# jeff-regier/Celeste.jl

Measured on AMD Instinct MI355X. Metric: sources/sec (ELBO value+gradient+Hessian+KL per target source), higher is better.
Workload: dtype f64; 1 GPU; BASELINE.json configs[2]: synthetic 2048x1489x5 SDSS-size field, 2000 star+galaxy sources, fp64, Sa=1 with value-only neighbours, psf_K=2; gather_backend=none, neighbor_links_rank0=3526

## Files before the change

### celeste.jl_amd/csrc/celeste_abi.hip

```cpp
#include <hip/hip_runtime.h>
#include <algorithm>
#include <atomic>
#include <cmath>
#include <cstdio>
#include <cstdlib>
#include <cstring>
#include <mutex>
#include <unordered_map>
#include <vector>

#include "elbo_kernels.h"
#include "optim_kernels.h"
#include "fused_kernels.h"
#include "host_tables.h"

struct celeste_group;

#define EVAL_FUSED_MAX 32

#define HIP_TRY(expr)                                                                    \
    do {                                                                                 \
        hipError_t e__ = (expr);                                                         \
        if (e__ != hipSuccess) {                                                         \
            fprintf(stderr, "celeste_mi355x: %s failed: %s (%s:%d)\n", #expr,            \
                    hipGetErrorString(e__), __FILE__, __LINE__);                         \
            return CELESTE_ERR_HIP;                                                      \
        }                                                                                \
    } while (0)

static hipError_t celeste_device_malloc(void **p, size_t bytes) {
    hipError_t e = (hipMalloc)(p, bytes);
    static const bool poison = [] { const char *v = getenv("CELESTE_POISON"); return v && atoi(v) != 0; }();
    if (e == hipSuccess && poison) {
        e = hipMemset(*p, 0xFF, bytes);
        if (e == hipSuccess) e = hipDeviceSynchronize();
    }
    return e;
}
#define hipMalloc(p, bytes) celeste_device_malloc((void **)(p), (bytes))

struct StreamPool {
    std::mutex mu;
    std::vector<hipStream_t> idle[16];
};
static StreamPool &stream_pool() { static StreamPool *p = new StreamPool(); return *p; }
static hipError_t stream_acquire(int device, hipStream_t *out) {
    *out = nullptr;
    if (device >= 0 && device < 16) {
        StreamPool &sp = stream_pool();
        std::lock_guard<std::mutex> lk(sp.mu);
        if (!sp.idle[device].empty()) { *out = sp.idle[device].back(); sp.idle[device].pop_back(); return hipSuccess; }
    }
    return hipStreamCreateWithFlags(out, hipStreamNonBlocking);
}
static void stream_retire(int device, hipStream_t s) {
    if (!s) return;
    if (hipStreamSynchronize(s) == hipSuccess && device >= 0 && device < 16) {
        static const size_t cap = [] { const char *e = getenv("CELESTE_STREAM_POOL_MAX"); return e ? (size_t)std::max(0, atoi(e)) : (size_t)32; }();
        StreamPool &sp = stream_pool();
        std::lock_guard<std::mutex> lk(sp.mu);
        if (sp.idle[device].size() < cap) { sp.idle[device].push_back(s); return; }
    } else (void)hipGetLastError();
    (void)hipStreamDestroy(s);
}

struct PinnedPool {
    std::mutex mu;
// ... 37 lines not shown


struct celeste_images {
    int device = 0;
    int N = 0;
    std::vector<DevImage> h_images;
    std::vector<void *> plane_allocs;
    DevImage *d_images = nullptr;
    std::atomic<int> refs{1};
};

static void images_release(celeste_images *im) {
    if (!im || im->refs.fetch_sub(1) != 1) return;
    (void)hipSetDevice(im->device);
    for (void *p : im->plane_allocs) (void)hipFree(p);
    if (im->d_images) (void)hipFree(im->d_images);
    delete im;
}

struct celeste_ctx {
    int device = 0;
    celeste_images *imgs = nullptr;
    hipStream_t stream = nullptr;
    hipStream_t copy_stream = nullptr;
    bool copy_stream_checked = false;
    int N = 0, S = 0, K = 0, NC = 0, n_stamps = 0;
    int chunk_px = 256, CH = 1;
    int max_npx = 0;
    std::vector<DevPatch> h_patches;
    std::vector<int64_t> h_nbr_off;
    std::vector<int32_t> h_nbr_idx;
    DevImage *d_images = nullptr;
    DevPatch *d_patches = nullptr;
    double *d_coefs = nullptr;
    float *d_coefs_f = nullptr;
    uint8_t *d_bitmaps = nullptr;
    int64_t *d_nbr_off = nullptr;
    int32_t *d_nbr_idx = nullptr;
    PriorDev *d_prior = nullptr;
    SrcImg *d_srcimg = nullptr;
    Comp *d_comps = nullptr;
    SrcGeo *d_geo = nullptr;
    int64_t *d_val_off = nullptr;
    double2 *d_val = nullptr;
    int32_t *d_needed = nullptr;
    int32_t stamp = 0;
    std::vector<int32_t> h_vis_off, h_vis_img, h_vis_src;
    int32_t *d_vis_off = nullptr, *d_vis_img = nullptr, *d_vis_src = nullptr;
    int4 *d_value_items = nullptr;
    int4 *d_vitems_src = nullptr;
    int32_t *d_vitem_off = nullptr;
    std::vector<int32_t> h_vitem_off;
    std::vector<int32_t> h_vitem_tgt;
    int64_t n_value_items = 0;
    std::vector<struct celeste_targets *> lists;
    int32_t *d_prep_mark = nullptr;
    double *d_lg_sum = nullptr;
    int64_t *d_nv_base = nullptr;
    int32_t *d_nbr_vis = nullptr;
    int2 *d_items = nullptr;
    size_t items_cap = 0;
    std::vector<int32_t> h_src_chunks;
    std::vector<int64_t> h_top_chunks;
    int max_src_chunks = 0;
    int32_t *d_work = nullptr, *d_work_blk = nullptr, *d_work_total = nullptr;
    size_t work_cap = 0, work_blk_cap = 0;
    int M = 1;
    bool dense = false;
    int64_t V = 0;
    std::vector<int64_t> h_tile_off;
    int64_t *d_tile_off = nullptr;
    int64_t n_tiles = 0;
    int sum_tiles = 4, RCH = 1;
    double *d_rec = nullptr;
    double *d_acc_split = nullptr;
    size_t acc_split_cap = 0;
    double *d_acc = nullptr;
    size_t acc_cap = 0;
    int32_t *d_rec_off = nullptr;
    size_t rec_off_cap = 0;
    double *d_vp = nullptr;
    int32_t *d_targets = nullptr;
    double *d_v = nullptr, *d_d = nullptr, *d_h = nullptr;
    int64_t *d_cnt = nullptr;
    int32_t *d_status = nullptr;
    size_t stage_cap = 0;
    double *p_vp = nullptr;
    int32_t *p_targets = nullptr, *p_status = nullptr;
    double *p_v = nullptr, *p_d = nullptr, *p_h = nullptr;
    int64_t *p_cnt = nullptr;
    size_t pin_cap = 0;
    double *d_small_in = nullptr, *p_small_in = nullptr, *d_small_out = nullptr, *p_small_out = nullptr;
    static const int MAX_PARTS = 8;
    hipEvent_t part_done[MAX_PARTS] = {}, part_copied[MAX_PARTS] = {};
    struct OptBuffers {
        size_t cap = 0;
        double *d_vp = nullptr, *d_v = nullptr, *d_d = nullptr, *d_h = nullptr, *d_H = nullptr, *d_T = nullptr, *d_S = nullptr, *d_pos = nullptr;
        int32_t *d_targets = nullptr, *d_act[2] = {nullptr, nullptr}, *d_evt[2] = {nullptr, nullptr}, *d_count = nullptr,
                *d_st = nullptr;
        void *d_state = nullptr;
        static const int RING = 4;
        double *h_vp = nullptr;
        void *h_state = nullptr;
        int32_t *h_count = nullptr;
        hipEvent_t ev[RING] = {};
    } opt;
// ... 340 lines not shown
        std::vector<int64_t> base((size_t)c->S + 1, 0);
        for (int s = 0; s < c->S; ++s)
            base[s + 1] = base[s] + (int64_t)(c->h_vis_off[s + 1] - c->h_vis_off[s]) * (c->h_nbr_off[s + 1] - c->h_nbr_off[s]);
        std::vector<int32_t> nv((size_t)base[c->S]);
        for (int s = 0; s < c->S; ++s) {
            const int64_t K = c->h_nbr_off[s + 1] - c->h_nbr_off[s];
            for (int v = c->h_vis_off[s]; v < c->h_vis_off[s + 1]; ++v)
                for (int64_t q = 0; q < K; ++q)
                    nv[base[s] + (int64_t)(v - c->h_vis_off[s]) * K + q] = (int32_t)hv(c->h_nbr_idx[c->h_nbr_off[s] + q], c->h_vis_img[v]);
        }
        CTX_TRY(dev_upload(&c->d_nv_base, base.data(), base.size()));
        CTX_TRY(dev_upload(&c->d_nbr_vis, nv.data(), nv.size()));
    }
    {
        std::vector<int32_t> sorted(c->h_src_chunks);
        std::sort(sorted.begin(), sorted.end(), [](int32_t a, int32_t b) { return a > b; });
        c->h_top_chunks.assign((size_t)c->S + 1, 0);
        for (int s = 0; s < c->S; ++s) c->h_top_chunks[s + 1] = c->h_top_chunks[s] + sorted[s];
    }
    CTX_TRY(dev_upload<int32_t>(&c->d_work_total, nullptr, 1));
    {
        if (c->N > 0xffff) { celeste_ctx_destroy(c); return CELESTE_ERR_INVALID_ARG; }
        const int n_cls = c->chunk_px / 64;
        std::vector<std::vector<std::pair<int32_t, int32_t>>> by_len(n_cls);
        for (int s = 0; s < c->S; ++s)
            for (int64_t q = c->h_nbr_off[s]; q < c->h_nbr_off[s + 1]; ++q) {
                const int s2 = c->h_nbr_idx[q];
                for (int va = c->h_vis_off[s]; va < c->h_vis_off[s + 1]; ++va) {
                    const int n = c->h_vis_img[va];
                    const int64_t vb = hv(s2, n);
                    if (vb < 0) continue;
                    const DevPatch &a = c->h_patches[va], &b = c->h_patches[vb];
                    const int rh = std::min(a.off_h + a.H2, b.off_h + b.H2) - std::max(a.off_h, b.off_h);
                    const int rw = std::min(a.off_w + a.W2, b.off_w + b.W2 - 1) - std::max(a.off_w, b.off_w);
                    if (rh <= 0 || rw <= 0) continue;
                    const int npx = rh * rw, nch = (npx + c->chunk_px - 1) / c->chunk_px;
                    for (int ch = 0; ch < nch; ++ch) {
                        const int px = std::min(c->chunk_px, npx - ch * c->chunk_px);
                        by_len[n_cls - (px + 63) / 64].push_back({(int32_t)q, (int32_t)(n | (ch << 16))});
                    }
                }
            }
        std::vector<int32_t> link_src(c->h_nbr_idx.size());
        for (int s = 0; s < c->S; ++s)
            for (int64_t q = c->h_nbr_off[s]; q < c->h_nbr_off[s + 1]; ++q) link_src[q] = s;
        std::vector<int4> desc;
        for (auto &v : by_len)
            for (auto &e : v) {
                const int t = link_src[e.first], s2 = c->h_nbr_idx[e.first], n = e.second & 0xffff, ch = e.second >> 16;
                desc.push_back(make_int4((int)hv(s2, n), (int)hv(t, n), ch, t));
            }
        c->n_value_items = (int64_t)desc.size();
        c->h_vitem_tgt.resize(desc.size());
        for (size_t i = 0; i < desc.size(); ++i) c->h_vitem_tgt[i] = desc[i].w;
        CTX_TRY(dev_upload(&c->d_value_items, desc.data(), desc.size()));
        c->h_vitem_off.assign((size_t)c->S + 1, 0);
        for (auto &d : desc) c->h_vitem_off[(size_t)d.w + 1]++;
        for (int s = 0; s < c->S; ++s) c->h_vitem_off[s + 1] += c->h_vitem_off[s];
        {
            std::vector<int4> by_src(desc.size());
            std::vector<int32_t> fill(c->h_vitem_off.begin(), c->h_vitem_off.end() - 1);
            for (auto &d : desc) by_src[(size_t)fill[d.w]++] = d;
            CTX_TRY(dev_upload(&c->d_vitems_src, by_src.data(), by_src.size()));
            CTX_TRY(dev_upload(&c->d_vitem_off, c->h_vitem_off.data(), c->h_vitem_off.size()));
        }
        CTX_TRY(dev_upload<int32_t>(&c->d_prep_mark, nullptr, (size_t)c->S));
        if (hipMemset(c->d_prep_mark, 0, (size_t)c->S * sizeof(int32_t)) != hipSuccess) { celeste_ctx_destroy(c); return CELESTE_ERR_HIP; }
    }
    {
        c->h_tile_off.resize(c->h_patches.size());
        int64_t tot = 0;
        for (size_t q = 0; q < c->h_patches.size(); ++q) {
            c->h_tile_off[q] = tot;
            tot += ((int64_t)c->h_patches[q].H2 * c->h_patches[q].W2 + 63) / 64;
        }
        c->n_tiles = tot;
        if (const char *e = getenv("CELESTE_SUM_TILES")) if (atoi(e) > 0) c->sum_tiles = atoi(e);
        c->RCH = std::max(1, ((c->max_npx + 63) / 64 + c->sum_tiles - 1) / c->sum_tiles);
    }
    if (hipStreamSynchronize(nullptr) != hipSuccess) { celeste_ctx_destroy(c); return CELESTE_ERR_HIP; }
#undef CTX_TRY
    *out = c;
    return CELESTE_OK;
} ABI_CATCH

static void targets_free(struct celeste_targets *t);
extern "C" void celeste_ctx_destroy(celeste_ctx_t *c) {
    if (!c) return;
    (void)hipSetDevice(c->device);
    if (c->stream) (void)hipStreamSynchronize(c->stream);
    if (c->copy_stream) (void)hipStreamSynchronize(c->copy_stream);
    for (struct celeste_targets *t : c->lists) targets_free(t);
    c->lists.clear();
    void *ptrs[] = {c->d_patches, c->d_coefs, c->d_coefs_f, c->d_bitmaps, c->d_nbr_off, c->d_nbr_idx, c->d_prior,
                    c->d_srcimg, c->d_comps, c->d_geo, c->d_val_off, c->d_val, c->d_needed, c->d_vis_off, c->d_vis_img, c->d_vis_src, c->d_value_items, c->d_vitems_src, c->d_vitem_off, c->d_prep_mark, c->d_rec_off, c->d_lg_sum, c->d_nv_base, c->d_nbr_vis, c->d_items, c->d_work, c->d_work_blk, c->d_work_total, c->d_tile_off, c->d_rec, c->d_acc_split, c->d_acc, c->d_vp, c->d_targets, c->d_v, c->d_d, c->d_h,
                    c->d_cnt, c->d_status};
    for (void *p : ptrs) if (p) (void)hipFree(p);
    {
        auto &o = c->opt;
        void *optr[] = {o.d_vp, o.d_v, o.d_d, o.d_h, o.d_H, o.d_T, o.d_S, o.d_pos, o.d_targets, o.d_act[0], o.d_act[1], o.d_evt[0], o.d_evt[1],
                        o.d_count, o.d_st, o.d_state};
        for (void *q : optr) if (q) (void)hipFree(q);
        void *hptr[] = {o.h_vp, o.h_state, o.h_count};
        for (void *q : hptr) if (q) staging_free(q);
        for (int k = 0; k < celeste_ctx::OptBuffers::RING; ++k) if (o.ev[k]) (void)hipEventDestroy(o.ev[k]);
        auto &f = c->fused;
        void *fptr[] = {f.d_chunk_desc, f.d_tgt_rec, f.d_q_items, f.d_q_ctl, f.d_arrivals, f.d_saved};
// ... 264 lines not shown
    d_active_rank, c->d_items, c->M, c->d_work, c->d_work_total, c->d_nv_base, c->d_nbr_vis, c->d_rec_off, c->d_coefs_f
#define LAUNCH_PIXEL_T(MODE, R) hipLaunchKernelGGL((pixel_kernel<MODE, R>), grid, dim3(64), 0, stream, PIXEL_ARGS)
#define LAUNCH_PIXEL_M(MODE) hipLaunchKernelGGL((pixel_kernel<MODE, double, true>), grid, dim3(64), 0, stream, PIXEL_ARGS)
#define LAUNCH_PIXEL(MODE) do { if (flags & CELESTE_FLAG_FP32) LAUNCH_PIXEL_T(MODE, float); else LAUNCH_PIXEL_T(MODE, double); } while (0)
    if (d_active_rank) {
        if (flags & CELESTE_FLAG_HESS) LAUNCH_PIXEL_M(2);
        else if (derivs) LAUNCH_PIXEL_M(1);
        else LAUNCH_PIXEL_M(0);
    }
    else if (split) LAUNCH_PIXEL(3);
    else if (flags & CELESTE_FLAG_HESS) LAUNCH_PIXEL(2);
    else if (derivs) LAUNCH_PIXEL(1);
    else LAUNCH_PIXEL_T(0, double);
#undef LAUNCH_PIXEL
#undef LAUNCH_PIXEL_M
#undef PIXEL_ARGS
#undef LAUNCH_PIXEL_T
    if (c->timing) HIP_TRY(hipEventRecord(c->ev[2], stream));
    c->ev_split = 0;
    const int lift_nt = n_targets <= 1024 ? 512 : 256;
    bool lift7 = n_targets > 4096;
    if (const char *e = getenv("CELESTE_LIFT_WAVES")) lift7 = atoi(e) == 7;
#define LAUNCH_LIFT(...) do { if (lift7) hipLaunchKernelGGL(lift_kernel<7>, __VA_ARGS__); else hipLaunchKernelGGL(lift_kernel<8>, __VA_ARGS__); } while (0)
    if (split) {
        hipLaunchKernelGGL(record_sum_kernel, dim3((unsigned)((size_t)n_targets * c->M * c->RCH)), dim3(RSUM_NT), 0,
                           stream, c->d_patches, d_targets, c->d_tile_off, reinterpret_cast<const double2 *>(c->d_rec),
                           c->d_items, c->N, c->M, c->RCH, c->sum_tiles, c->d_acc_split, nullptr, c->d_work_total);
        if (c->timing) { HIP_TRY(hipEventRecord(c->ev[4], stream)); c->ev_split = 1; }
        LAUNCH_LIFT(dim3(n_targets), dim3(lift_nt), 0, stream, d_vp, c->d_images, c->d_patches, c->d_geo,
                           c->d_nbr_off, c->d_nbr_idx, d_targets, c->d_acc_split, c->d_prior, c->d_vis_off, c->d_vis_img, c->N, c->M,
                           c->RCH, c->sum_tiles * 64, flags,
                           d_v, d_d, d_h, d_counters, d_status, d_live, d_active_rank ? nullptr : c->d_lg_sum, nullptr, d_h_pos);
    } else
    LAUNCH_LIFT(dim3(n_targets), dim3(lift_nt), 0, stream, d_vp, c->d_images, c->d_patches, c->d_geo,
                       c->d_nbr_off, c->d_nbr_idx, d_targets, c->d_acc, c->d_prior, c->d_vis_off, c->d_vis_img, c->N, c->M, CH,
                       chunk_px, flags,
                       d_v, d_d, d_h, d_counters, d_status, d_live, d_active_rank ? nullptr : c->d_lg_sum, c->d_rec_off, d_h_pos);
#undef LAUNCH_LIFT
    if (c->timing) { HIP_TRY(hipEventRecord(c->ev[3], stream)); c->ev_valid = 1; }
    HIP_TRY(hipGetLastError());
    return CELESTE_OK;
}

struct celeste_targets {
    celeste_ctx_t *ctx = nullptr;
    int32_t n = 0;
    int G = 1;
    int32_t *d_targets = nullptr;
    int32_t *d_work = nullptr, *d_work_total = nullptr, *d_rec_off = nullptr;
    int2 *d_items = nullptr;
    int32_t *d_needed = nullptr;
    int32_t *d_visits = nullptr;
    int32_t *d_vitems = nullptr;
    int64_t n_visits = 0, n_vitems = 0;
    int64_t n_records = 0;
    int32_t n_work = 0;
};
static const int32_t LIST_STAMP = 1;

static void targets_free(celeste_targets *t) {
    if (!t) return;
    void *ptrs[] = {t->d_targets, t->d_work, t->d_work_total, t->d_rec_off, t->d_items, t->d_needed, t->d_visits, t->d_vitems};
    for (void *p : ptrs) if (p) (void)hipFree(p);
    delete t;
}

static int targets_build(celeste_ctx_t *c, const std::vector<int32_t> &tg, celeste_targets_t **out) {
    const int32_t n = (int32_t)tg.size();
    if ((size_t)n * c->M * c->CH > 0x7fffffffull) return CELESTE_ERR_INVALID_ARG;
    HIP_TRY(hipSetDevice(c->device));
    celeste_targets *t = new celeste_targets;
    t->ctx = c; t->n = n; t->G = chunk_group(n);
    int32_t *d_blk = nullptr;
    auto fail = [&](int st) { if (d_blk) (void)hipFree(d_blk); (void)hipGetLastError(); targets_free(t); return st; };
#define LIST_TRY(expr) do { if ((expr) != hipSuccess) return fail(CELESTE_ERR_HIP); } while (0)
#define LIST_ALLOC(p, bytes) do { if (hipMalloc((void **)&(p), (bytes)) != hipSuccess) return fail(CELESTE_ERR_ALLOC); } while (0)
    std::vector<char> is_tgt((size_t)c->S, 0), reads((size_t)c->S, 0);
    for (int32_t s : tg) {
        is_tgt[s] = 1; reads[s] = 1;
        for (int64_t q = c->h_nbr_off[s]; q < c->h_nbr_off[s + 1]; ++q) reads[c->h_nbr_idx[q]] = 1;
        t->n_records += c->h_src_chunks[s];
    }
    std::vector<int32_t> visits, vitems;
    for (int s = 0; s < c->S; ++s)
        if (reads[s]) for (int v = c->h_vis_off[s]; v < c->h_vis_off[s + 1]; ++v) visits.push_back(v);
    for (size_t i = 0; i < c->h_vitem_tgt.size(); ++i) if (is_tgt[c->h_vitem_tgt[i]]) vitems.push_back((int32_t)i);
    t->n_visits = (int64_t)visits.size(); t->n_vitems = (int64_t)vitems.size();
    const int n_cand = n * c->M;
    const int n_wblk = (n_cand + WORK_NT - 1) / WORK_NT;
    const size_t n_blk = (size_t)n_wblk * (WORK_CLASSES + 1);
    LIST_ALLOC(t->d_targets, (size_t)n * sizeof(int32_t));
    LIST_ALLOC(t->d_work, std::max<size_t>((size_t)t->n_records, 1) * sizeof(int32_t));
    LIST_ALLOC(t->d_work_total, sizeof(int32_t));
    LIST_ALLOC(t->d_rec_off, (size_t)n_cand * sizeof(int32_t));
    if (!c->dense) LIST_ALLOC(t->d_items, (size_t)n_cand * sizeof(int2));
    LIST_ALLOC(t->d_needed, (size_t)c->S * sizeof(int32_t));
    LIST_ALLOC(t->d_visits, std::max<size_t>(visits.size(), 1) * sizeof(int32_t));
    LIST_ALLOC(t->d_vitems, std::max<size_t>(vitems.size(), 1) * sizeof(int32_t));
    LIST_ALLOC(d_blk, n_blk * sizeof(int32_t));
    LIST_TRY(hipMemcpy(t->d_targets, tg.data(), (size_t)n * sizeof(int32_t), hipMemcpyHostToDevice));
    if (!visits.empty()) LIST_TRY(hipMemcpy(t->d_visits, visits.data(), visits.size() * sizeof(int32_t), hipMemcpyHostToDevice));
    if (!vitems.empty()) LIST_TRY(hipMemcpy(t->d_vitems, vitems.data(), vitems.size() * sizeof(int32_t), hipMemcpyHostToDevice));
    LIST_TRY(hipMemset(t->d_needed, 0, (size_t)c->S * sizeof(int32_t)));
    const size_t setup_threads = (size_t)n * (c->dense ? 1 : c->M);
    hipLaunchKernelGGL(setup_kernel, dim3((unsigned)((setup_threads + 63) / 64)), dim3(64), 0, nullptr, (const double *)nullptr, -1,
                       (SrcGeo *)nullptr, t->d_targets, n, c->d_vis_off, c->d_vis_img, c->M, t->d_items, t->d_needed, LIST_STAMP,
                       (int32_t *)nullptr, c->d_nbr_off, c->d_nbr_idx, (const int32_t *)nullptr);
    hipLaunchKernelGGL(work_count_kernel, dim3(n_wblk), dim3(WORK_NT), 0, nullptr, t->d_targets, n_cand, c->d_patches,
                       c->d_vis_off, c->d_vis_img, c->N, c->M, c->chunk_px, t->G, (int)c->dense, d_blk, (const int32_t *)nullptr);
    hipLaunchKernelGGL(work_scan_kernel, dim3(1), dim3(1024), 0, nullptr, d_blk, (int)n_blk, t->d_work_total, n_wblk * WORK_CLASSES);
    hipLaunchKernelGGL(work_fill_kernel, dim3(n_wblk), dim3(WORK_NT), 0, nullptr, t->d_targets, n_cand, c->d_patches,
                       c->d_vis_off, c->d_vis_img, c->N, c->M, c->CH, c->chunk_px, t->G, (int)c->dense, d_blk, t->d_work,
                       (const int32_t *)nullptr, t->d_rec_off);
    LIST_TRY(hipGetLastError());
    LIST_TRY(hipMemcpy(&t->n_work, t->d_work_total, sizeof(int32_t), hipMemcpyDeviceToHost));
    LIST_TRY(hipFree(d_blk)); d_blk = nullptr;
#undef LIST_TRY
#undef LIST_ALLOC
    if (t->n_work < 0 || (int64_t)t->n_work > t->n_records) return fail(CELESTE_ERR_HIP);
    c->lists.push_back(t);
    *out = t;
    return CELESTE_OK;
}

extern "C" int celeste_targets_create(celeste_ctx_t *c, int32_t n_targets, const int32_t *targets, celeste_targets_t **out) try {
    if (!c || !out || !targets || n_targets <= 0) return CELESTE_ERR_INVALID_ARG;
    *out = nullptr;
    for (int32_t i = 0; i < n_targets; ++i) if (targets[i] < 0 || targets[i] >= c->S) return CELESTE_ERR_INVALID_ARG;
    return targets_build(c, std::vector<int32_t>(targets, targets + n_targets), out);
} ABI_CATCH

extern "C" int celeste_targets_create_device(celeste_ctx_t *c, int32_t n_targets, const int32_t *d_targets, void *stream_,
                                             celeste_targets_t **out) try {
    if (!c || !out || !d_targets || n_targets <= 0) return CELESTE_ERR_INVALID_ARG;
    *out = nullptr;
    HIP_TRY(hipSetDevice(c->device));
    std::vector<int32_t> tg((size_t)n_targets);
    HIP_TRY(hipMemcpyAsync(tg.data(), d_targets, (size_t)n_targets * sizeof(int32_t), hipMemcpyDeviceToHost, (hipStream_t)stream_));
    HIP_TRY(hipStreamSynchronize((hipStream_t)stream_));
    for (int32_t s : tg) if (s < 0 || s >= c->S) return CELESTE_ERR_INVALID_ARG;
    return targets_build(c, tg, out);
} ABI_CATCH

static void targets_release(celeste_targets_t *t) {
    celeste_ctx_t *c = t->ctx;
    auto it = std::find(c->lists.begin(), c->lists.end(), t);
    if (it != c->lists.end()) c->lists.erase(it);
    targets_free(t);
}

extern "C" void celeste_targets_destroy(celeste_targets_t *t) {
    if (!t) return;
    (void)hipSetDevice(t->ctx->device);
    (void)hipDeviceSynchronize();
    targets_release(t);
}

static int launch_prepared(celeste_ctx_t *c, const celeste_targets_t *t, const double *d_vp, uint32_t flags, double *d_v,
                           double *d_d, double *d_h, int64_t *d_counters, int32_t *d_status, void *stream_) {
    if (!c || !t || t->ctx != c) return CELESTE_ERR_INVALID_ARG;
    const int32_t n_targets = t->n;
    const char *off = getenv("CELESTE_NO_PREPARED");
    if ((off && atoi(off) != 0) || (flags & (CELESTE_FLAG_FP32 | CELESTE_FLAG_SPLIT)) ||
        want_eval_fused(flags, n_targets, true, d_d, d_h))
        return launch_eval(c, d_vp, n_targets, t->d_targets, flags, d_v, d_d, d_h, d_counters, d_status, stream_, true, nullptr,
                           t->n_records);
    if (!d_vp || !d_v || !d_status) return CELESTE_ERR_INVALID_ARG;
    if ((flags & CELESTE_FLAG_HESS) && !d_h) return CELESTE_ERR_INVALID_ARG;
    if ((flags & (CELESTE_FLAG_GRAD | CELESTE_FLAG_HESS)) && !d_d) return CELESTE_ERR_INVALID_ARG;
    hipStream_t stream = (hipStream_t)stream_;
    HIP_TRY(hipSetDevice(c->device));
    const size_t need = std::max<size_t>((size_t)t->n_records, 1) * ACC_N;
    if (need > c->acc_cap) {
        if (c->d_acc) { HIP_TRY(hipStreamSynchronize(stream)); HIP_TRY(hipFree(c->d_acc)); c->d_acc = nullptr; }
        HIP_TRY(hipMalloc((void **)&c->d_acc, need * sizeof(double)));
        c->acc_cap = need;
    }
    const int CH = c->CH, chunk_px = c->chunk_px;
    if (c->timing) HIP_TRY(hipEventRecord(c->ev[0], stream));
    const unsigned geo_blocks = (unsigned)((c->S + 63) / 64);
    hipLaunchKernelGGL(geo_prep_kernel, dim3(geo_blocks + (unsigned)t->n_visits), dim3(64), 0, stream, d_vp, c->d_images,
                       c->d_patches, c->d_vis_src, c->d_vis_img, c->K, c->d_srcimg, c->d_comps, t->d_visits, (int)geo_blocks,
                       c->S, c->d_geo);
    if (t->n_vitems > 0) {
        const bool wide_items = n_targets <= VALUE_WIDE_MAX && c->chunk_px == 256 && !getenv("CELESTE_NO_WIDE_VALUE");
#define LAUNCH_VALUE(WAVES)                                                                                                 \
        hipLaunchKernelGGL((value_kernel<double, WAVES>), dim3((unsigned)t->n_vitems), dim3(64 * WAVES), 0, stream,        \
                           c->d_patches, c->d_coefs, c->d_srcimg, c->d_comps, t->d_needed, LIST_STAMP, c->d_val_off,        \
                           c->d_value_items, c->NC, c->chunk_px, c->d_val, c->d_coefs_f, t->d_vitems)
        if (wide_items) LAUNCH_VALUE(4); else LAUNCH_VALUE(1);
#undef LAUNCH_VALUE
    }
    if (c->timing) HIP_TRY(hipEventRecord(c->ev[1], stream));
    const dim3 grid((unsigned)std::max<int32_t>(t->n_work, 1));
#define LAUNCH_PIXEL(MODE)                                                                                                  \
    hipLaunchKernelGGL((pixel_kernel<MODE, double>), grid, dim3(64), 0, stream, c->d_images, c->d_patches, c->d_coefs,      \
                       c->d_bitmaps, c->d_srcimg, c->d_comps, c->d_nbr_off, c->d_nbr_idx, c->d_val_off, c->d_val,           \
                       t->d_targets, c->N, c->NC, CH, chunk_px, t->G, c->d_acc, c->d_tile_off, c->d_rec,                    \
                       (const int32_t *)nullptr, t->d_items, c->M, t->d_work, t->d_work_total, c->d_nv_base, c->d_nbr_vis,  \
                       t->d_rec_off, c->d_coefs_f)
    if (flags & CELESTE_FLAG_HESS) LAUNCH_PIXEL(2);
    else if (flags & CELESTE_FLAG_GRAD) LAUNCH_PIXEL(1);
    else LAUNCH_PIXEL(0);
#undef LAUNCH_PIXEL
    if (c->timing) HIP_TRY(hipEventRecord(c->ev[2], stream));
    c->ev_split = 0;
    const int lift_nt = n_targets <= 1024 ? 512 : 256;
    bool lift7 = n_targets > 4096;
    if (const char *e = getenv("CELESTE_LIFT_WAVES")) lift7 = atoi(e) == 7;
#define LIFT_ARGS dim3(n_targets), dim3(lift_nt), 0, stream, d_vp, c->d_images, c->d_patches, c->d_geo, c->d_nbr_off,       \
                  c->d_nbr_idx, t->d_targets, c->d_acc, c->d_prior, c->d_vis_off, c->d_vis_img, c->N, c->M, CH, chunk_px,   \
                  flags, d_v, d_d, d_h, d_counters, d_status, (const int32_t *)nullptr, c->d_lg_sum, t->d_rec_off, \
                  (const int32_t *)nullptr
    if (lift7) hipLaunchKernelGGL(lift_kernel<7>, LIFT_ARGS); else hipLaunchKernelGGL(lift_kernel<8>, LIFT_ARGS);
#undef LIFT_ARGS
    if (c->timing) { HIP_TRY(hipEventRecord(c->ev[3], stream)); c->ev_valid = 1; }
    HIP_TRY(hipGetLastError());
    return CELESTE_OK;
}

extern "C" int celeste_elbo_eval_targets_device(celeste_ctx_t *c, const celeste_targets_t *t, const double *d_vp, uint32_t flags,
                                                double *d_v, double *d_d, double *d_h, int64_t *d_counters,
                                                int32_t *d_status, void *stream_) try {
    return launch_prepared(c, t, d_vp, flags, d_v, d_d, d_h, d_counters, d_status, stream_);
} ABI_CATCH

__global__ void spin_kernel(long long ticks) {
    const long long t0 = wall_clock64();
    while (wall_clock64() - t0 < ticks) __builtin_amdgcn_s_sleep(8);
}
static int pick_copy_stream(celeste_ctx_t *c) {
    if (c->copy_stream_checked) return CELESTE_OK;
    c->copy_stream_checked = true;
    if (const char *e = getenv("CELESTE_COPY_STREAM_CHECK")) if (atoi(e) == 0) return CELESTE_OK;
    const size_t bytes = 4u << 20;
    void *d_buf = nullptr, *h_buf = nullptr;
    hipEvent_t e0 = nullptr, e1 = nullptr;
// ... 1033 lines not shown
```

### celeste.jl_amd/csrc/elbo_kernels.h

```cpp
#pragma once
#include <hip/hip_runtime.h>
#include <math.h>
#include "elbo_device.h"
#include "../../include/celeste_mi355x.h"

#ifndef CELESTE_MUTANT
#define CELESTE_MUTANT 0
#endif

__constant__ double c_eta[16];
__constant__ double c_nu[16];

__device__ inline void bvn_cov(double ab, double angle, double scale, double &x11, double &x12, double &x22) {
    double sp, cp;
    sincos(angle, &sp, &cp);
    double ab_term = ab * ab - 1.0;
    double s2 = scale * scale;
    x12 = -s2 * cp * sp * ab_term;
    x11 = s2 * (1.0 + ab_term * (sp * sp));
    x22 = s2 * (1.0 + ab_term * (cp * cp));
}

__device__ inline void brightness(const double *vs, int i, int b, double &El, double &Ell) {
    const double r = vs[6 + i], v = vs[8 + i];
// ... 707 lines not shown
    const int lane = threadIdx.x & 63, wv = threadIdx.x >> 6;
    constexpr int NCL = WORK_CLASSES + 1;
    int cnt[NCL];
#pragma unroll
    for (int c = 0; c < NCL; ++c) cnt[c] = 0;
    for (int k = k0; k < k1; ++k) {
        int n_full, lc, nch;
        visit_chunks(k, targets, patches, vis_off, vis_img, N, M, chunk_px, G, dense != 0, n_full, lc, &nch);
        cnt[0] += n_full;
#pragma unroll
        for (int c = 1; c < WORK_CLASSES; ++c) cnt[c] += lc == c;
        cnt[WORK_CLASSES] += nch;
    }
    int off[NCL];
    if (threadIdx.x == 0) s_base[0] = 0;
#pragma unroll
    for (int c = 0; c < NCL; ++c) {
        int x = cnt[c];
#pragma unroll
        for (int d = 1; d < 64; d <<= 1) { const int y = __shfl_up(x, d); if (lane >= d) x += y; }
        __syncthreads();
        if (lane == 63) s_part[wv] = x;
        __syncthreads();
        int before = 0, tot = 0;
#pragma unroll
        for (int w = 0; w < WORK1_NT / 64; ++w) { const int v = s_part[w]; before += w < wv ? v : 0; tot += v; }
        off[c] = before + x - cnt[c];
        if (threadIdx.x == 0) s_base[c + 1] = s_base[c] + tot;
    }
    __syncthreads();
    if (threadIdx.x == 0) *work_total = s_base[WORK_CLASSES];
#pragma unroll
    for (int c = 0; c < WORK_CLASSES; ++c) off[c] += s_base[c];
    for (int k = k0; k < k1; ++k) {
        int n_full, lc, nch;
        visit_chunks(k, targets, patches, vis_off, vis_img, N, M, chunk_px, G, dense != 0, n_full, lc, &nch);
        for (int g = 0; g < n_full; ++g) work[off[0]++] = k * CH + g * G;
#pragma unroll
        for (int c = 1; c < WORK_CLASSES; ++c) if (lc == c) work[off[c]++] = k * CH + n_full * G;
        rec_off[k] = off[WORK_CLASSES];
        off[WORK_CLASSES] += nch;
    }
    if (fz_tgt_rec) {
        __syncthreads();
        for (int ti = threadIdx.x; ti < n_targets; ti += WORK1_NT) {
            int first;
            const int n_rec = describe_target_records(ti, targets[ti], patches, nullptr, N, M, fz_chunk_px, rec_off, fz_chunk_desc, first);
            fz_tgt_rec[ti] = make_int2(first < 0 ? 0 : first, n_rec);
        }
    }
}

template <bool COH, typename R = double>
__device__ __forceinline__ void value_pixels(int lane, const DevPatch &P, const SrcImg &si, const Comp *__restrict__ tc, int NC,
                                             const double *__restrict__ coefs, const double *__restrict__ etab, int h_lo,
                                             int w_lo, int RH, int p0, int p1, double2 *__restrict__ out,
                                             const float *__restrict__ tcf = nullptr) {
    const double *__restrict__ coef = coefs + (size_t)(CELESTE_MUTANT == 3 ? 0 : P.stamp) * (CEL_COEF * CEL_COEF);
    const double sh0 = 26.0 - si.m1, sw0 = 26.0 - si.m2;
    const float rRH = 1.0f / (float)RH;
    for (int idx = p0 + lane; idx < p1; idx += 64) {
        int rw, rh;
        divmod_small(idx, RH, rRH, rw, rh);
        const int h0 = h_lo + rh, w0 = w_lo + rw;
        const double hh = (double)(h0 + 1), ww = (double)(w0 + 1);
        double f0, f1;
        if constexpr (sizeof(R) == 8) {
            f0 = star_value(coef, hh + sh0, ww + sw0);
            f1 = galaxy_value(tc, NC, hh - si.m1, ww - si.m2, etab);
        } else {
            f0 = (double)star_value_f(coef, (float)(hh + sh0), (float)(ww + sw0));
            f1 = (double)galaxy_value_f(tcf, NC, (float)(hh - si.m1), (float)(ww - si.m2));
        }
        const double En = si.c0 * f0 + si.c1 * f1;
        const double E2n = si.q0 * (f0 * f0) + si.q1 * (f1 * f1);
        double2 *const o = out + ((h0 - P.off_h) + (int64_t)P.H2 * (w0 - P.off_w));
        const double var = E2n - En * En;
        if constexpr (COH) { stc<true>(&o->x, En); stc<true>(&o->y, var); }
        else *o = make_double2(En, var);
    }
}

typedef float f2v __attribute__((ext_vector_type(2)));
__device__ __forceinline__ void value_pixels_f2(int lane, const DevPatch &P, const SrcImg &si, int NC, const float *__restrict__ coef,
                                                int h_lo, int w_lo, int RH, int p0, int p1, double2 *__restrict__ out,
                                                const float *__restrict__ tcf) {
    const double sh0 = 26.0 - si.m1, sw0 = 26.0 - si.m2;
    const float rRH = 1.0f / (float)RH;
    const f2v *tp = reinterpret_cast<const f2v *>(tcf);
    const int n_dev = 8 * (NC / 14);
    for (int base = p0; base < p1; base += 128) {
        int h0[2], w0[2];
        bool ok[2];
        float dxs[2], dys[2], xh[2], xw[2];
#pragma unroll
        for (int q = 0; q < 2; ++q) {
            const int i = base + 64 * q + lane;
            ok[q] = i < p1;
            int rw, rh;
            divmod_small(min(i, p1 - 1), RH, rRH, rw, rh);
            h0[q] = h_lo + rh; w0[q] = w_lo + rw;
            const double hh = (double)(h0[q] + 1), ww = (double)(w0[q] + 1);
            dxs[q] = (float)(hh - si.m1); dys[q] = (float)(ww - si.m2);
            xh[q] = (float)(hh + sh0); xw[q] = (float)(ww + sw0);
        }
        const f2v dx = {dxs[0], dxs[1]}, dy = {dys[0], dys[1]};
        f2v f1 = (f2v)(0.0f);
        for (int c0 = 0; c0 < NC; c0 += (c0 < n_dev ? 8 : 6)) {
            const int len = c0 < n_dev ? 8 : 6;
            const f2v *k0 = tp + 3 * c0;
            const f2v d1 = dx - k0[3].xx, d2 = dy - k0[4].xx;
            const f2v s11 = -0.72134752044448170368f * (d1 * d1), s12 = -1.44269504088896340736f * (d1 * d2),
                      s22 = -0.72134752044448170368f * (d2 * d2);
            for (int c = c0; c < c0 + len; c += 2) {
                const f2v *k = tp + 3 * c;
                {
                    const f2v p11 = k[0].xx, p12 = k[1].xx, p22 = k[2].xx, w = k[5].xx;
                    const f2v q2 = p11 * s11 + (p12 * s12 + p22 * s22);
                    f1 += w * (f2v){__builtin_amdgcn_exp2f(q2.x), __builtin_amdgcn_exp2f(q2.y)};
                }
                {
#if CELESTE_MUTANT == 6
                    const f2v p11 = k[0].yy, p12 = k[1].xx, p22 = k[2].yy, w = k[5].yy;
#else
                    const f2v p11 = k[0].yy, p12 = k[1].yy, p22 = k[2].yy, w = k[5].yy;
#endif
                    const f2v q2 = p11 * s11 + (p12 * s12 + p22 * s22);
                    f1 += w * (f2v){__builtin_amdgcn_exp2f(q2.x), __builtin_amdgcn_exp2f(q2.y)};
                }
            }
        }
        const float *cc[2];
// ... 46 lines not shown
#endif
    const int4 it = items[item_list ? item_list[blockIdx.x] : blockIdx.x];
    const int sn = it.x, ch = it.z, t = it.w;
    if (is_target[t] != stamp) return;
    const DevPatch &P = patches[sn];
    const DevPatch &T = patches[it.y];
    const int h_lo = max(P.off_h, T.off_h), h_hi = min(P.off_h + P.H2, T.off_h + T.H2);
    const int w_lo = max(P.off_w, T.off_w), w_hi = min(P.off_w + P.W2 - 1, T.off_w + T.W2);
    const int RH = h_hi - h_lo, RW = w_hi - w_lo;
    if (RH <= 0 || RW <= 0) return;
    const int npx = RH * RW;
    const int p0 = ch * chunk_px;
    if (p0 >= npx) return;
    VT(0);
    exp_table_init(etab);
    const int p1 = min(npx, p0 + chunk_px);
    const SrcImg si = srcimg[sn];
    __shared__ Comp tc[14 * CEL_MAXK];
    {
        const double *src = reinterpret_cast<const double *>(comps + (size_t)sn * NC);
        double *dst = reinterpret_cast<double *>(tc);
        for (int i = threadIdx.x; i < NC * 8; i += 64 * WAVES) dst[i] = src[i];
        __syncthreads();
    }
    __shared__ float tcf[sizeof(R) == 4 ? 6 * 14 * CEL_MAXK : 2];
    if constexpr (sizeof(R) == 4) {
        if ((int)threadIdx.x < NC) {
            const Comp k = tc[threadIdx.x];
            float *o = tcf + 12 * (threadIdx.x >> 1) + (threadIdx.x & 1);
            o[0] = (float)k.p11; o[2] = (float)k.p12; o[4] = (float)k.p22; o[6] = (float)k.xi1; o[8] = (float)k.xi2; o[10] = (float)k.w0;
        }
        __syncthreads();
    }
    VT(1);
    if constexpr (sizeof(R) == 4) {
        const int q0 = p0 + 128 * (int)(threadIdx.x >> 6);
        if (WAVES == 1 || q0 < p1)
            value_pixels_f2(threadIdx.x & 63, P, si, NC, coefs_f + (size_t)(CELESTE_MUTANT == 3 ? 0 : P.stamp) * (CEL_COEF * CEL_COEF), h_lo, w_lo, RH,
                            WAVES == 1 ? p0 : q0, WAVES == 1 ? p1 : min(p1, q0 + 128), val + val_off[sn], tcf);
    } else if constexpr (WAVES == 1)
        value_pixels<false, R>(threadIdx.x, P, si, tc, NC, coefs, etab, h_lo, w_lo, RH, p0, p1, val + val_off[sn], tcf);
    else {
        const int q0 = p0 + 64 * (int)(threadIdx.x >> 6);
        if (q0 < p1) value_pixels<false, R>(threadIdx.x & 63, P, si, tc, NC, coefs, etab, h_lo, w_lo, RH, q0, min(p1, q0 + 64), val + val_off[sn], tcf);
    }
    VT(2);
#ifdef VALUE_TIMING
    if (threadIdx.x == 0) {
        for (int k = 0; k < 3; ++k) atomicAdd(&g_value_clk[k], (unsigned long long)(vts[k + 1] - vts[k]));
        atomicAdd(&g_value_clk[7], 1ull); atomicAdd(&g_value_clk[6], (unsigned long long)((p1 - p0 + 63) / 64));
    }
#endif
#undef VT
}

template <typename S>
struct PixelTermsT {
    typedef S scalar;
    S vterm, cnt_act, cnt_inact;
    S f0, f1;
    S alpha, beta, w2, w12;
    S k0, k1;
    S f0g0, f0g1, f0h0, f0h1, f0h2;
    S C0s, C0g, C1s, C1g;
    S Q0s, Q0g, Q1s, Q1g;
    S Wgg, Wsg, Wss;
    S S0d, S1x, S1y, S1xd, S1yd, S2a, S2b, S2c, S2an, S2bn, S2cn, S2ad, S2bd, S2cd;
    S S3a, S3b, S3c, S3d, S4a, S4b, S4c, S4d, S4e;
};
typedef PixelTermsT<double> PixelTerms;

template <int G, class TT>
__device__ __forceinline__ typename TT::scalar gal_g(const TT &T) {
    typedef typename TT::scalar S;
    if constexpr (G == 0) return T.S1x;
    else if constexpr (G == 1) return T.S1y;
    else if constexpr (G == 2) return T.S0d;
    else if constexpr (G == 3) return (S)0.5 * T.S2an;
    else if constexpr (G == 4) return T.S2bn;
    else return (S)0.5 * T.S2cn;
}
template <int G, int G2, class TT>
__device__ __forceinline__ typename TT::scalar gal_h(const TT &T) {
    typedef typename TT::scalar S;
    constexpr int k = G * 6 + G2;
    if constexpr (k == 0) return T.S2a;
    else if constexpr (k == 1) return T.S2b;
    else if constexpr (k == 2) return T.S1xd;
    else if constexpr (k == 3) return (S)0.5 * T.S3a;
    else if constexpr (k == 4) return T.S3b;
    else if constexpr (k == 5) return (S)0.5 * T.S3c;
    else if constexpr (k == 7) return T.S2c;
    else if constexpr (k == 8) return T.S1yd;
    else if constexpr (k == 9) return (S)0.5 * T.S3b;
    else if constexpr (k == 10) return T.S3c;
    else if constexpr (k == 11) return (S)0.5 * T.S3d;
    else if constexpr (k == 14) return (S)0.0;
    else if constexpr (k == 15) return (S)0.5 * T.S2ad;
    else if constexpr (k == 16) return T.S2bd;
    else if constexpr (k == 17) return (S)0.5 * T.S2cd;
    else if constexpr (k == 21) return (S)0.25 * T.S4a;
    else if constexpr (k == 22) return (S)0.5 * T.S4b;
    else if constexpr (k == 23) return (S)0.25 * T.S4c;
    else if constexpr (k == 28) return T.S4c;
    else if constexpr (k == 29) return (S)0.5 * T.S4d;
    else { static_assert(k == 35, "upper triangle only"); return (S)0.25 * T.S4e; }
// ... 1809 lines not shown
```

Baseline: 3.169 million sources/sec.

## Deduplicate neighbour value pixels via per-visit union of target overlaps

Builds, per target list, the union of pixels each value-only neighbour visit must supply across all targets it overlaps. These are stored as compact pixel offset lists chunked into work items. A new value_union_kernel evaluates each unique pixel once instead of once per (neighbour, target) link, removing redundant star/galaxy evaluations where target patches overlap. It adds host-side preprocessing at list build and an indirect offset load per pixel, and the old path is kept behind an environment variable.

```diff
diff --git a/celeste.jl_amd/csrc/celeste_abi.hip b/celeste.jl_amd/csrc/celeste_abi.hip
--- a/celeste.jl_amd/csrc/celeste_abi.hip
+++ b/celeste.jl_amd/csrc/celeste_abi.hip
@@ -13,6 +13,7 @@
 #include "optim_kernels.h"
 #include "fused_kernels.h"
 #include "host_tables.h"
+#include "value_union.h"
 
 struct celeste_group;
 
@@ -156,6 +157,7 @@
     int32_t *d_vitem_off = nullptr;
     std::vector<int32_t> h_vitem_off;
     std::vector<int32_t> h_vitem_tgt;
+    std::vector<ValueUnionLink> h_vitem_link;
     int64_t n_value_items = 0;
     std::vector<struct celeste_targets *> lists;
     int32_t *d_prep_mark = nullptr;
@@ -602,7 +604,8 @@
             }
         c->n_value_items = (int64_t)desc.size();
         c->h_vitem_tgt.resize(desc.size());
-        for (size_t i = 0; i < desc.size(); ++i) c->h_vitem_tgt[i] = desc[i].w;
+        c->h_vitem_link.resize(desc.size());
+        for (size_t i = 0; i < desc.size(); ++i) { c->h_vitem_tgt[i] = desc[i].w; c->h_vitem_link[i] = {desc[i].x, desc[i].y}; }
         CTX_TRY(dev_upload(&c->d_value_items, desc.data(), desc.size()));
         c->h_vitem_off.assign((size_t)c->S + 1, 0);
         for (auto &d : desc) c->h_vitem_off[(size_t)d.w + 1]++;
@@ -973,7 +976,9 @@
     int32_t *d_needed = nullptr;
     int32_t *d_visits = nullptr;
     int32_t *d_vitems = nullptr;
-    int64_t n_visits = 0, n_vitems = 0;
+    int4 *d_uitems = nullptr;
+    int32_t *d_upx = nullptr;
+    int64_t n_visits = 0, n_vitems = 0, n_uitems = 0;
     int64_t n_records = 0;
     int32_t n_work = 0;
 };
@@ -981,7 +986,8 @@
 
 static void targets_free(celeste_targets *t) {
     if (!t) return;
-    void *ptrs[] = {t->d_targets, t->d_work, t->d_work_total, t->d_rec_off, t->d_items, t->d_needed, t->d_visits, t->d_vitems};
+    void *ptrs[] = {t->d_targets, t->d_work, t->d_work_total, t->d_rec_off, t->d_items, t->d_needed, t->d_visits, t->d_vitems,
+                    t->d_uitems, t->d_upx};
     for (void *p : ptrs) if (p) (void)hipFree(p);
     delete t;
 }
@@ -1006,7 +1012,18 @@
     for (int s = 0; s < c->S; ++s)
         if (reads[s]) for (int v = c->h_vis_off[s]; v < c->h_vis_off[s + 1]; ++v) visits.push_back(v);
     for (size_t i = 0; i < c->h_vitem_tgt.size(); ++i) if (is_tgt[c->h_vitem_tgt[i]]) vitems.push_back((int32_t)i);
-    t->n_visits = (int64_t)visits.size(); t->n_vitems = (int64_t)vitems.size();
+    std::vector<int32_t> upx;
+    std::vector<ValueUnionItem> uitems;
+    {
+        static_assert(sizeof(ValueUnionBox) == 4 * sizeof(int32_t) && sizeof(ValueUnionItem) == sizeof(int4), "layout");
+        std::vector<ValueUnionBox> boxes(c->h_patches.size());
+        for (size_t v = 0; v < boxes.size(); ++v) { const DevPatch &q = c->h_patches[v]; boxes[v] = {q.off_h, q.off_w, q.H2, q.W2}; }
+        std::vector<ValueUnionLink> links;
+        links.reserve(vitems.size());
+        for (int32_t i : vitems) links.push_back(c->h_vitem_link[(size_t)i]);
+        if (!value_union_build(boxes.data(), std::move(links), c->chunk_px, upx, uitems)) return fail(CELESTE_ERR_INVALID_ARG);
+    }
+    t->n_visits = (int64_t)visits.size(); t->n_vitems = (int64_t)vitems.size(); t->n_uitems = (int64_t)uitems.size();
     const int n_cand = n * c->M;
     const int n_wblk = (n_cand + WORK_NT - 1) / WORK_NT;
     const size_t n_blk = (size_t)n_wblk * (WORK_CLASSES + 1);
@@ -1018,10 +1035,14 @@
     LIST_ALLOC(t->d_needed, (size_t)c->S * sizeof(int32_t));
     LIST_ALLOC(t->d_visits, std::max<size_t>(visits.size(), 1) * sizeof(int32_t));
     LIST_ALLOC(t->d_vitems, std::max<size_t>(vitems.size(), 1) * sizeof(int32_t));
+    LIST_ALLOC(t->d_uitems, std::max<size_t>(uitems.size(), 1) * sizeof(int4));
+    LIST_ALLOC(t->d_upx, std::max<size_t>(upx.size(), 1) * sizeof(int32_t));
     LIST_ALLOC(d_blk, n_blk * sizeof(int32_t));
     LIST_TRY(hipMemcpy(t->d_targets, tg.data(), (size_t)n * sizeof(int32_t), hipMemcpyHostToDevice));
     if (!visits.empty()) LIST_TRY(hipMemcpy(t->d_visits, visits.data(), visits.size() * sizeof(int32_t), hipMemcpyHostToDevice));
     if (!vitems.empty()) LIST_TRY(hipMemcpy(t->d_vitems, vitems.data(), vitems.size() * sizeof(int32_t), hipMemcpyHostToDevice));
+    if (!uitems.empty()) LIST_TRY(hipMemcpy(t->d_uitems, uitems.data(), uitems.size() * sizeof(int4), hipMemcpyHostToDevice));
+    if (!upx.empty()) LIST_TRY(hipMemcpy(t->d_upx, upx.data(), upx.size() * sizeof(int32_t), hipMemcpyHostToDevice));
     LIST_TRY(hipMemset(t->d_needed, 0, (size_t)c->S * sizeof(int32_t)));
     const size_t setup_threads = (size_t)n * (c->dense ? 1 : c->M);
     hipLaunchKernelGGL(setup_kernel, dim3((unsigned)((setup_threads + 63) / 64)), dim3(64), 0, nullptr, (const double *)nullptr, -1,
@@ -1103,7 +1124,18 @@
     hipLaunchKernelGGL(geo_prep_kernel, dim3(geo_blocks + (unsigned)t->n_visits), dim3(64), 0, stream, d_vp, c->d_images,
                        c->d_patches, c->d_vis_src, c->d_vis_img, c->K, c->d_srcimg, c->d_comps, t->d_visits, (int)geo_blocks,
                        c->S, c->d_geo);
-    if (t->n_vitems > 0) {
+    const char *no_union = getenv("CELESTE_NO_VALUE_UNION");
+    if (!(no_union && atoi(no_union) != 0)) {
+        if (t->n_uitems > 0) {
+            const bool wide_items = n_targets <= VALUE_WIDE_MAX && c->chunk_px == 256 && !getenv("CELESTE_NO_WIDE_VALUE");
+#define LAUNCH_UNION(WAVES)                                                                                                 \
+            hipLaunchKernelGGL((value_union_kernel<WAVES>), dim3((unsigned)t->n_uitems), dim3(64 * WAVES), 0, stream,       \
+                               c->d_patches, c->d_coefs, c->d_srcimg, c->d_comps, c->d_val_off, t->d_uitems, t->d_upx,      \
+                               c->NC, c->d_val)
+            if (wide_items) LAUNCH_UNION(4); else LAUNCH_UNION(1);
+#undef LAUNCH_UNION
+        }
+    } else if (t->n_vitems > 0) {
         const bool wide_items = n_targets <= VALUE_WIDE_MAX && c->chunk_px == 256 && !getenv("CELESTE_NO_WIDE_VALUE");
 #define LAUNCH_VALUE(WAVES)                                                                                                 \
         hipLaunchKernelGGL((value_kernel<double, WAVES>), dim3((unsigned)t->n_vitems), dim3(64 * WAVES), 0, stream,        \
diff --git a/celeste.jl_amd/csrc/elbo_kernels.h b/celeste.jl_amd/csrc/elbo_kernels.h
--- a/celeste.jl_amd/csrc/elbo_kernels.h
+++ b/celeste.jl_amd/csrc/elbo_kernels.h
@@ -783,6 +783,28 @@
 }
 
 template <bool COH, typename R = double>
+__device__ __forceinline__ void value_pixel(const DevPatch &P, const SrcImg &si, const Comp *__restrict__ tc, int NC,
+                                            const double *__restrict__ coef, const double *__restrict__ etab, double sh0,
+                                            double sw0, int h0, int w0, double2 *__restrict__ out,
+                                            const float *__restrict__ tcf = nullptr) {
+    const double hh = (double)(h0 + 1), ww = (double)(w0 + 1);
+    double f0, f1;
+    if constexpr (sizeof(R) == 8) {
+        f0 = star_value(coef, hh + sh0, ww + sw0);
+        f1 = galaxy_value(tc, NC, hh - si.m1, ww - si.m2, etab);
+    } else {
+        f0 = (double)star_value_f(coef, (float)(hh + sh0), (float)(ww + sw0));
+        f1 = (double)galaxy_value_f(tcf, NC, (float)(hh - si.m1), (float)(ww - si.m2));
+    }
+    const double En = si.c0 * f0 + si.c1 * f1;
+    const double E2n = si.q0 * (f0 * f0) + si.q1 * (f1 * f1);
+    double2 *const o = out + ((h0 - P.off_h) + (int64_t)P.H2 * (w0 - P.off_w));
+    const double var = E2n - En * En;
+    if constexpr (COH) { stc<true>(&o->x, En); stc<true>(&o->y, var); }
+    else *o = make_double2(En, var);
+}
+
+template <bool COH, typename R = double>
 __device__ __forceinline__ void value_pixels(int lane, const DevPatch &P, const SrcImg &si, const Comp *__restrict__ tc, int NC,
                                              const double *__restrict__ coefs, const double *__restrict__ etab, int h_lo,
                                              int w_lo, int RH, int p0, int p1, double2 *__restrict__ out,
@@ -793,22 +815,7 @@
     for (int idx = p0 + lane; idx < p1; idx += 64) {
         int rw, rh;
         divmod_small(idx, RH, rRH, rw, rh);
-        const int h0 = h_lo + rh, w0 = w_lo + rw;
-        const double hh = (double)(h0 + 1), ww = (double)(w0 + 1);
-        double f0, f1;
-        if constexpr (sizeof(R) == 8) {
-            f0 = star_value(coef, hh + sh0, ww + sw0);
-            f1 = galaxy_value(tc, NC, hh - si.m1, ww - si.m2, etab);
-        } else {
-            f0 = (double)star_value_f(coef, (float)(hh + sh0), (float)(ww + sw0));
-            f1 = (double)galaxy_value_f(tcf, NC, (float)(hh - si.m1), (float)(ww - si.m2));
-        }
-        const double En = si.c0 * f0 + si.c1 * f1;
-        const double E2n = si.q0 * (f0 * f0) + si.q1 * (f1 * f1);
-        double2 *const o = out + ((h0 - P.off_h) + (int64_t)P.H2 * (w0 - P.off_w));
-        const double var = E2n - En * En;
-        if constexpr (COH) { stc<true>(&o->x, En); stc<true>(&o->y, var); }
-        else *o = make_double2(En, var);
+        value_pixel<COH, R>(P, si, tc, NC, coef, etab, sh0, sw0, h_lo + rh, w_lo + rw, out, tcf);
     }
 }
 
@@ -961,6 +968,60 @@
     }
 #endif
 #undef VT
+}
+
+template <int WAVES = 1>
+__global__ void __launch_bounds__(64 * WAVES)
+value_union_kernel(const DevPatch *__restrict__ patches, const double *__restrict__ coefs,
+                   const SrcImg *__restrict__ srcimg, const Comp *__restrict__ comps, const int64_t *__restrict__ val_off,
+                   const int4 *__restrict__ items, const int32_t *__restrict__ px_off, int NC, double2 *__restrict__ val) {
+    __shared__ double etab[64];
+    const int4 it = items[blockIdx.x];
+    const int sn = it.x, count = it.z;
+    const int32_t *__restrict__ po = px_off + it.y;
+    const int lane = threadIdx.x & 63;
+    int o0 = 0, o1 = 0, o2 = 0, o3 = 0;
+    if constexpr (WAVES == 1) {
+        if (lane < count) o0 = po[lane];
+        if (lane + 64 < count) o1 = po[lane + 64];
+        if (lane + 128 < count) o2 = po[lane + 128];
+        if (lane + 192 < count) o3 = po[lane + 192];
+    } else if ((int)threadIdx.x < count) o0 = po[threadIdx.x];
+    const DevPatch &P = patches[sn];
+    exp_table_init(etab);
+    const SrcImg si = srcimg[sn];
+    __shared__ Comp tc[14 * CEL_MAXK];
+    {
+        const double *src = reinterpret_cast<const double *>(comps + (size_t)sn * NC);
+        double *dst = reinterpret_cast<double *>(tc);
+        for (int i = threadIdx.x; i < NC * 8; i += 64 * WAVES) dst[i] = src[i];
+        __syncthreads();
+    }
+    const double *__restrict__ coef = coefs + (size_t)(CELESTE_MUTANT == 3 ? 0 : P.stamp) * (CEL_COEF * CEL_COEF);
+    const double sh0 = 26.0 - si.m1, sw0 = 26.0 - si.m2;
+    const int H2 = P.H2;
+    const float rH2 = 1.0f / (float)H2;
+    double2 *__restrict__ out = val + val_off[sn];
+    if constexpr (WAVES == 1) {
+        for (int base = 0;;) {
+            const int n = min(count - base, 256);
+            for (int p = lane; p < n; p += 64) {
+                int cw, ch;
+                divmod_small(o0, H2, rH2, cw, ch);
+                o0 = o1; o1 = o2; o2 = o3;
+                value_pixel<false, double>(P, si, tc, NC, coef, etab, sh0, sw0, P.off_h + ch, P.off_w + cw, out);
+            }
+            base += 256;
+            if (base >= count) break;
+            const int i = base + lane;
+            o0 = i < count ? po[i] : 0; o1 = i + 64 < count ? po[i + 64] : 0;
+            o2 = i + 128 < count ? po[i + 128] : 0; o3 = i + 192 < count ? po[i + 192] : 0;
+        }
+    } else if ((int)threadIdx.x < count) {
+        int cw, ch;
+        divmod_small(o0, H2, rH2, cw, ch);
+        value_pixel<false, double>(P, si, tc, NC, coef, etab, sh0, sw0, P.off_h + ch, P.off_w + cw, out);
+    }
 }
 
 template <typename S>
diff --git a/celeste.jl_amd/csrc/value_union.h b/celeste.jl_amd/csrc/value_union.h
--- /dev/null
+++ b/celeste.jl_amd/csrc/value_union.h
@@ -0,0 +1,46 @@
+#pragma once
+#include <algorithm>
+#include <cstddef>
+#include <cstdint>
+#include <vector>
+
+struct ValueUnionBox { int32_t off_h, off_w, H2, W2; };
+struct ValueUnionLink { int32_t vb, va; };
+struct ValueUnionItem { int32_t vb, first, count, trips; };
+
+inline bool value_union_build(const ValueUnionBox *boxes, std::vector<ValueUnionLink> links, int chunk_px,
+                              std::vector<int32_t> &offsets, std::vector<ValueUnionItem> &items) {
+    offsets.clear(); items.clear();
+    std::sort(links.begin(), links.end(), [](const ValueUnionLink &a, const ValueUnionLink &b) {
+        return a.vb != b.vb ? a.vb < b.vb : a.va < b.va;
+    });
+    links.erase(std::unique(links.begin(), links.end(), [](const ValueUnionLink &a, const ValueUnionLink &b) {
+        return a.vb == b.vb && a.va == b.va;
+    }), links.end());
+    const int n_cls = chunk_px / 64;
+    std::vector<std::vector<ValueUnionItem>> by_len((size_t)std::max(n_cls, 1));
+    std::vector<unsigned char> wanted;
+    for (size_t i = 0; i < links.size();) {
+        const int32_t vb = links[i].vb;
+        const ValueUnionBox &b = boxes[vb];
+        const size_t npx = b.H2 > 0 && b.W2 > 0 ? (size_t)b.H2 * (size_t)b.W2 : 0;
+        wanted.assign(npx, 0);
+        for (; i < links.size() && links[i].vb == vb; ++i) {
+            const ValueUnionBox &a = boxes[links[i].va];
+            const int64_t h_lo = std::max(a.off_h, b.off_h), h_hi = std::min((int64_t)a.off_h + a.H2, (int64_t)b.off_h + b.H2);
+            const int64_t w_lo = std::max(a.off_w, b.off_w), w_hi = std::min((int64_t)a.off_w + a.W2, (int64_t)b.off_w + b.W2 - 1);
+            for (int64_t w = w_lo; w < w_hi; ++w)
+                for (int64_t h = h_lo; h < h_hi; ++h) wanted[(size_t)((h - b.off_h) + (int64_t)b.H2 * (w - b.off_w))] = 1;
+        }
+        const size_t first = offsets.size();
+        for (size_t p = 0; p < npx; ++p) if (wanted[p]) offsets.push_back((int32_t)p);
+        const size_t count = offsets.size() - first;
+        if (offsets.size() > (size_t)INT32_MAX) { offsets.clear(); items.clear(); return false; }
+        for (size_t p0 = 0; p0 < count; p0 += (size_t)chunk_px) {
+            const int32_t px = (int32_t)std::min((size_t)chunk_px, count - p0), trips = (px + 63) / 64;
+            by_len[(size_t)(n_cls - trips)].push_back({vb, (int32_t)(first + p0), px, trips});
+        }
+    }
+    for (auto &v : by_len) items.insert(items.end(), v.begin(), v.end());
+    return true;
+}
```

Result: faster. 3.231 million sources/sec (median of 6 runs) (+1.9%).
